# GianniLunardi/VBOC

Hardware: AMD Instinct MI355X
Metric: VBOC boundary OCP solves/sec, triple pendulum, 1/2/4/8 MI355X (higher is better)
Workload: dtype f64

## Files before the change

vboc_amd/csrc/coop.h:

```cpp
#pragma once

#ifndef VBOC_NSF
#define VBOC_NSF 4
#endif
#ifndef VBOC_DF
#define VBOC_DF 2
#endif
#ifndef VBOC_NSV
#define VBOC_NSV 8
#endif
#ifndef VBOC_DV
#define VBOC_DV 6
#endif

namespace vboc {

typedef double dbl2 __attribute__((ext_vector_type(2)));
typedef double dbl4 __attribute__((ext_vector_type(4)));
typedef __attribute__((address_space(1))) dbl2 gdbl2;
typedef __attribute__((address_space(1))) void gvoid;
typedef __attribute__((address_space(3))) void lvoid;

__host__ __device__ constexpr int even_up(int v) { return (v + 1) & ~1; }
#ifndef VBOC_REC_ALIGN
// ... 172 lines not shown
#else
#define CPROF_DECL
#define CPROF(i)
#define CPROF_FLUSH(sq, ip)
#endif
#if defined(VBOC_COOP_PROF) && defined(VBOC_PROF_SPLIT)
#define SPROF_DECL(P) unsigned long long sp0 = 0, sp1 = 0, sp2 = 0, sp3 = 0, sp4 = 0, sp_t = 0; \
  constexpr bool sp_on = (VBOC_PROF_SPLIT == (P)); if (sp_on) sp_t = __builtin_amdgcn_s_memtime();
#define SPROF(i) if (sp_on) { const unsigned long long n_ = __builtin_amdgcn_s_memtime(); sp##i += n_ - sp_t; sp_t = n_; }
#define SPROF_FLUSH if (sp_on && t == 0) { atomicAdd(&g_wave_prof[11], sp0); atomicAdd(&g_wave_prof[12], sp1); \
  atomicAdd(&g_wave_prof[13], sp2); atomicAdd(&g_wave_prof[14], sp3); atomicAdd(&g_wave_prof[15], sp4); }
#else
#define SPROF_DECL(P)
#define SPROF(i)
#define SPROF_FLUSH
#endif
#ifndef VBOC_REPEAT
#define VBOC_REPEAT 0
#endif

#define VREP(id, stmt) do { stmt; if constexpr (VBOC_REPEAT == (id)) { stmt; } } while (0)

#ifndef VBOC_FUSE
#define VBOC_FUSE 31
#endif

template <int NQ, bool FM = false, bool HC = false>
struct Coop {
  using L = WaveLayout<NQ>;
  using HL = Lane<NQ>;
  static_assert(!HC || (!FM && NQ >= 2 && NQ <= 3), "path constraint: pendulum chains, VALU factorisation");
  using PF = Par<NQ>;
  static constexpr int NX = 2 * NQ, NU = NQ, NZ = 3 * NQ, M0 = NQ + 1, REC = L::REC;
  static constexpr bool FUSE_OK = FM && NQ <= 3 && !HC;
  static constexpr bool FAC1 = FUSE_OK && (VBOC_FUSE & 1), PFUSE = FUSE_OK && (VBOC_FUSE & 2),
                        CCORR = FUSE_OK && (VBOC_FUSE & 4), KFM = FUSE_OK && (VBOC_FUSE & 8);
  static constexpr int OA = L::OA, OB = L::OB, OZ = L::OZ, ODZ = L::ODZ, OQL = L::OQL, OQU = L::OQU,
                       OE = L::OE, OK = L::OK, OKF = L::OKF, OLR = L::OLR, OM = L::OM, OY = L::OY,
                       OPE = L::OPE, OD = L::OD, ODA = L::ODA, OC = L::OC, OACL = L::OACL, OX = L::OX, OU = L::OU,
                       OPI = L::OPI,
                       OLL = L::OLL, OLU = L::OLU, OWPI = L::OWPI;

  double* s;
  gdouble* g;
  const Work& w;
  const Opts& o;
  int t;
  int N;
  double rs, rd0, e00, mu, nbox;

  unsigned lds0;
  gdouble* gh = nullptr;
  int pause_at = -1;

  __device__ Coop(double* s_, gdouble* g_, const Work& w_, const Opts& o_, int t_)
      : s(s_), g(g_), w(w_), o(o_), t(t_), N(0),
        lds0((unsigned)__builtin_amdgcn_readfirstlane((int)(unsigned)(size_t)(lvoid*)s_)) {}

  __device__ __forceinline__ void fresh() { asm volatile("" : "+v"(t)); }
// ... 104 lines not shown
  __device__ __forceinline__ double cgrad(int k, int i) const { return (k == 0 && i == 0) ? par(PF::CS) : 0.0; }

  template <int LO, int C>
  __device__ __forceinline__ void ldr(int k, double (&d)[2 * C]) const {
    static_assert(LO % 2 == 0, "16-byte aligned range");
    const gdbl2* src = (const gdbl2*)(g + (long long)k * REC + LO);
    UNR for (int c = 0; c < C; ++c) {
      const dbl2 v = src[c];
      d[2 * c] = v.x;
      d[2 * c + 1] = v.y;
    }
  }
  static constexpr int NIP = (4 * NZ + 1) / 2;
  struct IP { double v[2 * NIP]; };
  __device__ __forceinline__ void ld_ip(int k, IP& r) const { ldr<OZ, NIP>(k, r.v); }
  template <int LO, int CNT, bool WIDE = !L::IN_FIRST>
  struct Cov {
    static_assert(LO >= OD && LO + CNT <= OD + 2 * NZ, "a part of the D / DA slots");
    static constexpr int B = WIDE ? OD : (LO & ~1), OFF = LO - B, C = WIDE ? (2 * NZ + 1) / 2 : (OFF + CNT + 1) / 2;
    double v[2 * C];
  };
  template <int LO, int CNT>
  __device__ __forceinline__ void ldc(int k, Cov<LO, CNT>& c) const { ldr<Cov<LO, CNT>::B, Cov<LO, CNT>::C>(k, c.v); }

  struct CS { double tl, tu, itl, itu, ql, qu, dz; bool bx; };
  __device__ __forceinline__ CS comp_r(const IP& r, int k, int i) const {
    CS c;
    double lb, ub;
    c.bx = box(k, i, lb, ub);
    const double z = r.v[i];
    c.dz = r.v[NZ + i]; c.ql = r.v[2 * NZ + i]; c.qu = r.v[3 * NZ + i];
    c.tl = c.dz - (lb - z); c.tu = (ub - z) - c.dz;
    c.itl = c.bx ? 1.0 / c.tl : 0.0;
    c.itu = c.bx ? 1.0 / c.tu : 0.0;
    return c;
  }
  __device__ __forceinline__ CS comp(int k, int i) const {
    CS c;
    double lb, ub;
    c.bx = box(k, i, lb, ub);
    const double z = st(k, OZ + i);
    c.dz = st(k, ODZ + i); c.ql = st(k, OQL + i); c.qu = st(k, OQU + i);
    c.tl = c.dz - (lb - z); c.tu = (ub - z) - c.dz;
    c.itl = c.bx ? 1.0 / c.tl : 0.0;
    c.itu = c.bx ? 1.0 / c.tu : 0.0;
    return c;
// ... 421 lines not shown
    for (int k = t; k <= N; k += 64) {
      IP r;
      ld_ip(k, r);
      __builtin_amdgcn_sched_barrier(0);
      gdouble* rec = &g[(long long)k * REC];
      prep_from(r, k, rec);
      if constexpr (HC) {
        if (hc_on(k)) {
          const double htl = hcr(k, HL::HTL), htu = hcr(k, HL::HTU), hql = hcr(k, HL::HQL), hqu = hcr(k, HL::HQU);
          const double sig = hql / htl + hqu / htu;
          const double gam = hql * (rs * hcr(k, HL::HR0L)) / htl - hqu * (rs * hcr(k, HL::HR0U)) / htu;
          double hg[NQ];
          UNR for (int j = 0; j < NQ; ++j) hg[j] = hcr(k, HL::HG + j);
          UNR for (int i = 0; i < NQ; ++i) {
            UNR for (int j = 0; j < NQ; ++j)
              rec[OK + i * NQ + j] = (i == j ? (double)rec[OD + i] : 0.0) + sig * hg[i] * hg[j];
            rec[ODA + i] += hg[i] * gam;
          }
        }
      }
    }
    __syncthreads();
  }
  __device__ __forceinline__ void prep_corr(double smu) {
    fresh();
    for (int k = t; k <= N; k += 64) {
      IP r;
      Cov<ODA, NZ> da;
      ld_ip(k, r);
      ldc(k, da);
      __builtin_amdgcn_sched_barrier(0);
      gdouble* rec = &g[(long long)k * REC];
      double gv[NZ];
      UNR for (int i = 0; i < NZ; ++i) {
        const CS c = comp_r(r, k, i);
        double gg = o.lm * c.dz + cgrad(k, i);
        if (c.bx) {
          double rl, ru;
          corr_rhs(c, da.v[da.OFF + i], smu, rl, ru);
          gg += -c.ql - rl * c.itl + c.qu + ru * c.itu;
        }
        rec[OD + i] = gg;
        gv[i] = gg;
      }
      if constexpr (CCORR) {
        if (k >= 1 && k < N) vec_const(k, gv);
      }
      if constexpr (HC) {
// ... 578 lines not shown
        double x = st(0, OG + a);
        UNR for (int i = 0; i < NX; ++i) x += s[L::F0 + i * M0 + a] * v[i];
        w0[a] = x;
      }
      UNR for (int e = 0; e < M0 * M0; ++e) Lm[e] = s[L::LR0 + e];
      chol_solve<M0>(Lm, w0);
      UNR for (int a = 0; a < M0; ++a) w0[a] = -w0[a];
      UNR for (int j = 0; j < NQ; ++j)
        UNR for (int a = 0; a < M0; ++a) lin[j] += s[L::Y0 + a * NQ + j] * w0[a];
    }
    double Sl[NQ * NQ];
    UNR for (int e = 0; e < NQ * NQ; ++e) Sl[e] = s[L::SC + e];
    const bool ok = chol<NQ>(Sl);
    UNR for (int j = 0; j < NQ; ++j) nun[j] = lin[j] + s[L::LINE + j] - rs * par(PF::E0N + j);
    chol_solve<NQ>(Sl, nun);
    __syncthreads();
    SPROF(3)
    SPROF_FLUSH
    return ok;
  }

  template <bool CORR>
  __device__ __forceinline__ void fwd(const double (&w0in)[M0], const double (&nun)[NQ], double smu, double& amax, double& c0,
                      double& c1, double& c2) {
    fresh();
    constexpr int OT = CORR ? OD : ODA;
#if defined(VBOC_PROF_SPLIT) && VBOC_PROF_SPLIT == 6
    constexpr int WSPL = 6;
#else
    constexpr int WSPL = 3;
#endif
#define W3(i) if constexpr (WSPL == 3) { SPROF(i) }
#define W6(i) if constexpr (WSPL == 6) { SPROF(i) }
    SPROF_DECL(WSPL)
    {
      double w0[M0];
      UNR for (int a = 0; a < M0; ++a) {
        double x = w0in[a];
        UNR for (int j = 0; j < NQ; ++j) x -= s[L::MM0 + a * NQ + j] * nun[j];
        w0[a] = x;
      }
      if (t == 0) {
        UNR for (int i = 0; i < NZ; ++i) st(0, OT + i) = i < M0 ? w0[i < M0 ? i : 0] : 0.0;

      }
      if (t < NX) {
        double x = rs * st(0, OE + t);
// ... 101 lines not shown
        const int k = 1 + j;
        wdma(j + L::DV);
        vmwait<(L::DV - 1) * PW>();
        double an[NX], cn;
        fld(vslot((j + 1) % L::NSV), an, cn);
        __builtin_amdgcn_sched_barrier(0);
        double p0 = cc, p1 = 0.0;
        UNR for (int q = 0; q < NX; q += 2) p0 += acl[q] * dx[q];
        UNR for (int q = 1; q < NX; q += 2) p1 += acl[q] * dx[q];
        const double dn = p0 + p1;
        if (t < NX) s[L::XS + (k + 1) * NX + t] = dn;
        UNR for (int q = 0; q < NX; ++q) dx[q] = rdlane(dn, q);
        UNR for (int q = 0; q < NX; ++q) acl[q] = an[q];
        cc = cn;
      }
    }
    }
    __syncthreads();
    W3(2)
    W6(4)
    typename Lane<NQ>::MinRatio mr{1.0, CORR ? o.tau : 1.0};
    double a0 = 0.0, a1 = 0.0, a2 = 0.0;
    constexpr int NKM = KFM ? (OKF + NU - OK + 1) / 2 : (OY - OK + 1) / 2;
    for (int k = t; k <= N; k += 64) {
      IP r;
      double km[2 * NKM];
      Cov<ODA, NZ> da;
      const int kk = (k > 0 && k < N) ? k : 1 < N ? 1 : 0;
      ld_ip(k, r);
      ldr<OK, NKM>(kk, km);
      if (CORR) ldc(k, da);
      __builtin_amdgcn_sched_barrier(0);
      W6(0)
      gdouble* rec = &g[(long long)k * REC];
      double d[NZ];
      if (k == 0) {
        UNR for (int i = 0; i < NZ; ++i) d[i] = rec[OT + i];
      } else {
        UNR for (int i = 0; i < NX; ++i) d[i] = s[L::XS + k * NX + i];
        UNR for (int a = 0; a < NU; ++a) {
          double x = 0.0;
          if (k < N) {
            x = km[OKF - OK + a];
            if constexpr (!KFM) {
              UNR for (int j = 0; j < NQ; ++j) x -= km[OM - OK + a * NQ + j] * nun[j];
            }
// ... 34 lines not shown
            hcr(k, HL::HATL) = dtl; hcr(k, HL::HATU) = dtu; hcr(k, HL::HAQL) = dql; hcr(k, HL::HAQU) = dqu;
            a0 += htl * hql + htu * hqu;
            a1 += htl * dql + dtl * hql + htu * dqu + dtu * hqu;
            a2 += dtl * dql + dtu * dqu;
          }
          mr.add(htl, dtl);
          mr.add(htu, dtu);
          mr.add(hql, dql);
          mr.add(hqu, dqu);
        }
      }
      W6(2)
    }
    amax = wmind(mr.value());
    c0 = wsum(a0); c1 = wsum(a1); c2 = wsum(a2);
    __syncthreads();
    W3(3)
    W6(3)
    SPROF_FLUSH
#undef W3
#undef W6
  }

  __device__ __forceinline__ void update(double alpha, double smu) {
    fresh();
    double musum = 0.0;
    for (int k = t; k <= N; k += 64) {
      IP r;
      double dd[2 * ((2 * NZ + 1) / 2)];
      ld_ip(k, r);
      ldr<OD, (2 * NZ + 1) / 2>(k, dd);
      __builtin_amdgcn_sched_barrier(0);
      gdouble* rec = &g[(long long)k * REC];
      IP rn;
      if constexpr (PFUSE) rn = r;
      UNR for (int i = 0; i < NZ; ++i) {
        const CS c = comp_r(r, k, i);
        const double d = dd[i];
        const double dzn = c.dz + alpha * d;
        rec[ODZ + i] = dzn;
        if constexpr (PFUSE) rn.v[NZ + i] = dzn;
        if (!c.bx) continue;
        double rl, ru;
        corr_rhs(c, dd[NZ + i], smu, rl, ru);
        const double dll = (rl - c.ql * d) * c.itl, dlu = (ru + c.qu * d) * c.itu;
        const double qln = c.ql + alpha * dll, qun = c.qu + alpha * dlu;
        rec[OQL + i] = qln;
// ... 233 lines not shown
      else if (rstat < o.tol_stat && req < o.tol_eq && rineq < o.tol_ineq && rcomp < o.tol_comp) status = 0;
      else if (it >= o.max_iter) status = 2;
      if (status >= 0) break;
      qp_init();
      CPROF(1)
      int qcur = 0, qst = 1;
      double w0[M0], nun[NQ];
      for (;;) {
        int q = qp_check();
        if (q == 1 && qcur >= o.qp_max_iter) q = 2;
        if (q != 1) { qst = q; break; }
        if (!PFUSE || qcur == 0) VREP(1, prep_pred());
        CPROF(2)
        bool okf;
        if constexpr (FM) VREP(2, okf = factor_mfma());
        else VREP(2, okf = factor());
        if constexpr (!ACL_FUSED) VREP(3, acl_pass());
        CPROF(3)
        bool okv;
        VREP(4, (okv = vec<ODA, true, VFUSE>(w0, nun)));
        CPROF(4)
        if (!(okf && okv)) { qst = -1; break; }
        double aa, c0, c1, c2;
        VREP(5, fwd<false>(w0, nun, 0.0, aa, c0, c1, c2));
        CPROF(5)
        const double muaff = (c0 + aa * (c1 + aa * c2)) / nbox;
        double sig = muaff / mu;
        sig = fmin(1.0, sig * sig * sig);
        const double smu = sig * mu;
        VREP(6, prep_corr(smu));
        CPROF(2)
        bool okc;
        VREP(7, (okc = vec<OD, !CCORR>(w0, nun)));
        if (!okc) { qst = -1; break; }
        CPROF(4)
        double amax;
        VREP(8, fwd<true>(w0, nun, smu, amax, c0, c1, c2));
        CPROF(5)
        const double alpha = fmin(1.0, o.tau * amax);
        update(alpha, smu);
        if (t == 0) {
          UNR for (int j = 0; j < NQ; ++j) par(PF::QNU + j) += alpha * (nun[j] - par(PF::QNU + j));
        }
        __syncthreads();
        rs *= (1.0 - alpha);
        ++qcur;
        CPROF(6)
      }
      qit += qcur;
      qtot += qcur;
      if (qst < 0 || !costate()) { status = 4; break; }
      CPROF(7)
      update_weights();
      double alpha = 1.0;
      const double phi0 = merit(0.0);
      for (;;) {
        const double pa = merit(alpha);
        if (pa < phi0) break;
        if (alpha * o.alpha_red < o.alpha_min) break;
        alpha *= o.alpha_red;
      }
      apply(alpha);
      CPROF(8)
// ... 54 lines not shown
            in.sqp_iter[pid] = 0;
            in.qp_iter[pid] = 0;
            atomicAdd(ss.done, 1u);
          }
          continue;
        }
      }
      C.from_inputs(in, pid);
    }
    const int status = C.run(it, qit);
    C.store(in, pid, status, it, qit);
    __syncthreads();
    if (t == 0) {
      if (jb.list) {
        ss(IS_PID, slot) = -1;
        ss(IS_PH, slot) = 0;
      }
      atomicAdd(ss.done, 1u);
    }
  }
  if constexpr (NQ == 3 && FM && !HC && Coop<NQ, FM, HC>::VFUSE) asm volatile(".rept 96\n\ts_nop 0\n\t.endr");
}

__global__ void k_list(SlotState ss, int* list, unsigned* cnt) {
  const unsigned slot = blockIdx.x * blockDim.x + threadIdx.x;
  if (ss(IS_PID, slot) >= 0 && ss(IS_PH, slot) == 1) list[atomicAdd(cnt, 1u)] = (int)slot;
}

}
```

vboc_amd/csrc/dg.h:

```cpp
#pragma once

namespace vboc {

struct DgJobs {
  const long long* ids;
  int count;
  int N_start, nmax;
  int fail_mod;
  int max_restarts;
  double fmt_scale;
  unsigned long long seed;
  double q_min, q_max, v_max, u_max, dt, tol, eps, g, l1, l2, m1, m2;
  double* xs;
  double* us;
  double* vr;
  double* st;
  int vr_cap, st_doubles;
  double* rows;
  long long rows_cap;
  long long* row_off;
  int* row_cnt;
  double* ic;
  int* ic_slot;
  double* stats;
// ... 899 lines not shown
    const int e = ld_flag(&J->park_q[(long long)q * J->count + h]);
    if (e > 0 && (unsigned)(e - 1) / (unsigned)J->round_n < r) return true;
  }
  return false;
}
template <int NQ>
__device__ __forceinline__ bool dg_restart_before(const DgJobs* J, unsigned r) {
  const unsigned h = __hip_atomic_load(J->spec_q_head, __ATOMIC_RELAXED, __HIP_MEMORY_SCOPE_AGENT);
  if (h >= __hip_atomic_load(J->spec_q_tail, __ATOMIC_RELAXED, __HIP_MEMORY_SCOPE_AGENT)) return false;
  const int e = ld_flag(&J->spec_q[h]);
  if (e <= 0) return false;
  after_flag();
  const int ev = (e - 1) / (DG_SPEC_JOBS + 1);
  const double job = ld_coh(J->spec + (long long)ev * J->spec_stride + Dg<NQ>::H_JOB);
  return (unsigned)job / (unsigned)J->round_n < r;
}

template <int NQ, bool FM>
__global__ __launch_bounds__(64) __attribute__((amdgpu_waves_per_eu(WavesPerEu<NQ>::v, WavesPerEu<NQ>::v)))
void k_dg(Work w, Opts o, Inputs in, const Inputs* inp, const DgJobs* J, WaveJobs jb) {
  extern __shared__ __attribute__((aligned(16))) double smem[];
  const int t = (int)threadIdx.x;
  const int wg = (int)blockIdx.x;
  Coop<NQ, FM> C(smem, gptr(jb.regions) + (long long)wg * jb.region_doubles, w, o, t);
  const int count = J->count;
  const bool spec = J->spec_events > 0;
  const bool park = J->park_res != nullptr;
  if (spec && J->spec_crit && t == 0) {
    unsigned long long z = 0;
    __hip_atomic_compare_exchange_strong(J->t_launch, &z, (unsigned long long)__builtin_amdgcn_s_memrealtime(),
                                         __ATOMIC_RELAXED, __ATOMIC_RELAXED, __HIP_MEMORY_SCOPE_AGENT);
  }
  for (;;) {
    int mode = 0, idx = 0, ev = 0, jj = 0, code = 0;
    if (spec && (J->spec_window > 0 || J->spec_crit)) {
      int got = -1;
      if (t == 0) {
        const unsigned h = __hip_atomic_load(J->spec_eq_head, __ATOMIC_RELAXED, __HIP_MEMORY_SCOPE_AGENT);
        unsigned hh = h;
        if (h < __hip_atomic_load(J->spec_eq_tail, __ATOMIC_RELAXED, __HIP_MEMORY_SCOPE_AGENT) &&
            __hip_atomic_compare_exchange_strong(J->spec_eq_head, &hh, h + 1, __ATOMIC_RELAXED, __ATOMIC_RELAXED,
                                                 __HIP_MEMORY_SCOPE_AGENT)) {
          int e;
          while ((e = ld_flag(&J->spec_eq[h])) == 0) __builtin_amdgcn_s_sleep(2);
          after_flag();
          const int ev_ = (e - 1) / (DG_SPEC_JOBS + 1), jj_ = (e - 1) % (DG_SPEC_JOBS + 1);
          if (ld_flag(&J->spec_cancel[ev_]) == 0 &&
// ... 381 lines not shown

template <int NQ>
__device__ __forceinline__ bool ts_start(const DgJobs* J, const Inputs* in, int wg, int t, int job) {
  Ts<NQ> T(*J, *in, wg, t);
  return T.start(job);
}
template <int NQ>
__device__ __forceinline__ int ts_feed(const DgJobs* J, const Inputs* in, int wg, int t, int job) {
  Ts<NQ> T(*J, *in, wg, t);
  return T.feed(job);
}
template <int NQ>
__device__ __forceinline__ void ts_finish(const DgJobs* J, const Inputs* in, int wg, int t, int job) {
  Ts<NQ> T(*J, *in, wg, t);
  T.finish(job);
}

template <int NQ, bool FM>
__global__ __launch_bounds__(64) __attribute__((amdgpu_waves_per_eu(WavesPerEu<NQ>::v, WavesPerEu<NQ>::v)))
void k_ts(Work w, Opts o, Inputs in, const Inputs* inp, const DgJobs* J, WaveJobs jb) {
  extern __shared__ __attribute__((aligned(16))) double smem[];
  const int t = (int)threadIdx.x;
  const int wg = (int)blockIdx.x;
  Coop<NQ, FM> C(smem, gptr(jb.regions) + (long long)wg * jb.region_doubles, w, o, t);
  const int count = J->count;
  for (;;) {
    int got = -1;
    if (t == 0 && __hip_atomic_load(jb.next, __ATOMIC_RELAXED, __HIP_MEMORY_SCOPE_AGENT) < (unsigned)count) {
      const unsigned i = atomicAdd(jb.next, 1u);
      if (i < (unsigned)count) got = (int)i;
    }
    got = dg_bcast(got);
    if (got < 0) break;
    int code = ts_start<NQ>(J, inp, wg, t, got) ? 1 : 0;
    while (code) {
      __syncthreads();
      int it = 0, qit = 0;
      Lane<NQ> chk(w, o, 0u);
      if (!chk.supported(in, wg)) {
        if (t == 0) {
          in.status[wg] = 5;
          in.sqp_iter[wg] = 0;
          in.qp_iter[wg] = 0;
        }
      } else {
        C.from_inputs(in, wg);
        const int status = C.run(it, qit);
// ... 228 lines not shown
```

vboc_amd/csrc/vboc_solver.hip:

```cpp
#include <hip/hip_runtime.h>

#include <chrono>
#include <cmath>
#include <cstdlib>
#include <cstdio>
#include <cstring>
#include <string>
#include <vector>

#include "../../include/vboc.h"
#include "model.h"

#define UNR _Pragma("unroll")
#ifdef VBOC_WAVES
#define VBOC_WPE __attribute__((amdgpu_waves_per_eu(VBOC_WAVES, VBOC_WAVES)))
#else
#define VBOC_WPE
#endif

namespace vboc {

struct Opts {
  double tol_stat, tol_eq, tol_ineq, tol_comp;
  double qp_tol_stat, qp_tol_eq, qp_tol_comp;
// ... 1317 lines not shown
  int nq, nmax, device;
  long long slots;
  Opts o;
  Work w;
  void* pool = nullptr;
  size_t pool_bytes = 0;
  unsigned int* head = nullptr;
  int* ist = nullptr;
  unsigned int* host_done = nullptr;
  hipEvent_t ev0 = nullptr, ev1 = nullptr;
  int launches = 0;
  bool profile = false;
  std::vector<hipEvent_t> pev;
  int npev = 0;
  double fact_ms = 0.0;
  long long fact_calls = 0;
  unsigned long long fact_stages = 0;
  void* stage = nullptr;
  size_t stage_bytes = 0;
  int* list = nullptr;
  double coop_threshold = 8192;
  bool wave_all = true;
  bool factor_mfma = true;
  double* regions = nullptr;
  long long n_regions = 0, region_doubles = 0, group_cap = 0;
  double mall_mib = 256.0;
  size_t wave_lds = 0;
  bool coop_ok = false;
  long long coop_count = 0;
  double* ft_regions = nullptr;
  size_t ft_bytes = 0;
  double* dg_scratch = nullptr;
  size_t dg_bytes = 0;
  DgJobs* dg_jobs = nullptr;
  Inputs* dg_in = nullptr;
  TtJobs* tt_jobs = nullptr;
  bool tt_attr[2] = {false, false};
  bool dg_attr[4] = {false, false, false, false};
  int dg_fail_mod = 0;
  bool dg_speculate = true;
  int dg_spec_early = 0;
  int dg_spec_pause = 300;
  int dg_spec_first = 2;
  bool dg_spec_crit = false;
  int dg_spec_window = 0;
  double* wave_hc = nullptr;
// ... 112 lines not shown
    h->ft_bytes = need;
  }
  if constexpr (NQ == 3) {
    if (mp.on) {
      hipLaunchKernelGGL((k_ft<NQ, true>), dim3((unsigned)groups), dim3(64), 0, st, h->o, in, h->ft_regions, rd, h->head,
                         mp);
      return hipGetLastError() == hipSuccess ? 0 : -2;
    }
  }
  if (mp.on) return -2;
  hipLaunchKernelGGL((k_ft<NQ, false>), dim3((unsigned)groups), dim3(64), 0, st, h->o, in, h->ft_regions, rd, h->head,
                     mp);
  return hipGetLastError() == hipSuccess ? 0 : -2;
}

static long long wave_group_budget(const vboc_solver* h, int nmax) {
  const long long hot = (long long)(h->nq == 1 ? WaveLayout<1>::OX
                                    : (h->nq == 2 ? WaveLayout<2>::OX : (h->nq == 3 ? WaveLayout<3>::OX : WaveLayout<4>::OX))) *
                        (long long)(nmax + 1) * (long long)sizeof(double);
  const long long g = (long long)(0.92 * h->mall_mib * 1024.0 * 1024.0) / (hot > 0 ? hot : 1);
  return g < 256 ? 256 : g;
}

static hipError_t launch_wave(vboc_solver* h, const WaveJobs& jb, long long jobs, hipStream_t st, const Work& w,
                              const Inputs& in, const SlotState& ss) {
  long long groups = jobs < h->n_regions ? jobs : h->n_regions;
  const long long cap = h->group_cap > 0 ? h->group_cap : (h->mall_mib > 0 ? wave_group_budget(h, in.nmax) : 0);
  if (cap > 0 && groups > cap) groups = cap;
  if (groups < 1) return hipSuccess;
  h->last_groups = groups;
  const dim3 grid((unsigned)groups), block(64);
  switch (h->nq) {
    case 1:
      if (h->factor_mfma) hipLaunchKernelGGL((k_wave<1, true>), grid, block, h->wave_lds, st, w, h->o, in, ss, jb);
      else hipLaunchKernelGGL((k_wave<1, false>), grid, block, h->wave_lds, st, w, h->o, in, ss, jb);
      break;
    case 2:
      if (h->o.hc) hipLaunchKernelGGL((k_wave<2, false, true>), grid, block, h->wave_lds, st, w, h->o, in, ss, jb);
      else if (h->factor_mfma) hipLaunchKernelGGL((k_wave<2, true>), grid, block, h->wave_lds, st, w, h->o, in, ss, jb);
      else hipLaunchKernelGGL((k_wave<2, false>), grid, block, h->wave_lds, st, w, h->o, in, ss, jb);
      break;
    case 3:
      if (h->factor_mfma) hipLaunchKernelGGL((k_wave<3, true>), grid, block, h->wave_lds, st, w, h->o, in, ss, jb);
      else hipLaunchKernelGGL((k_wave<3, false>), grid, block, h->wave_lds, st, w, h->o, in, ss, jb);
      break;
    default: hipLaunchKernelGGL((k_wave<4, false>), grid, block, h->wave_lds, st, w, h->o, in, ss, jb); break;
  }
  return hipGetLastError();
}

template <int NQ, bool FM>
static hipError_t launch_dg(vboc_solver* h, const DgJobs& J, const Inputs& in, long long groups, hipStream_t st,
                           bool testing = false) {
  const void* fn = testing ? (const void*)k_ts<NQ, FM> : (const void*)k_dg<NQ, FM>;
  bool& attr = h->dg_attr[(FM ? 1 : 0) + (testing ? 2 : 0)];
  if (!attr) {
    hipError_t e = hipFuncSetAttribute(fn, hipFuncAttributeMaxDynamicSharedMemorySize, (int)h->wave_lds);
    if (e != hipSuccess) return e;
    attr = true;
  }
  WaveJobs jb{nullptr, J.count, J.next, h->regions, h->region_doubles};
  hipError_t e = hipMemcpyAsync(h->dg_jobs, &J, sizeof(DgJobs), hipMemcpyHostToDevice, st);
  if (e == hipSuccess) e = hipMemcpyAsync(h->dg_in, &in, sizeof(Inputs), hipMemcpyHostToDevice, st);
  if (e == hipSuccess) e = hipStreamSynchronize(st);
  if (e != hipSuccess) return e;
  if (testing)
// ... 157 lines not shown
  if (!h || !f) return fail(VBOC_ERR_ARG, "vboc_set_option: NULL argument");
  Opts& o = h->o;
  const std::string s(f);
  if (s == "nlp_solver_tol_stat") o.tol_stat = v;
  else if (s == "nlp_solver_tol_eq") o.tol_eq = v;
  else if (s == "nlp_solver_tol_ineq") o.tol_ineq = v;
  else if (s == "nlp_solver_tol_comp") o.tol_comp = v;
  else if (s == "nlp_solver_max_iter") o.max_iter = (int)v;
  else if (s == "qp_solver_iter_max") o.qp_max_iter = (int)v;
  else if (s == "qp_solver_tol_stat") o.qp_tol_stat = v;
  else if (s == "qp_solver_tol_eq") o.qp_tol_eq = v;
  else if (s == "qp_solver_tol_comp") o.qp_tol_comp = v;
  else if (s == "levenberg_marquardt") o.lm = v;
  else if (s == "alpha_min") o.alpha_min = v;
  else if (s == "alpha_reduction") o.alpha_red = v;
  else if (s == "ipm_mu0") o.mu0 = v;
  else if (s == "ipm_push") o.push = v;
  else if (s == "ipm_tau") o.tau = v;
  else if (s == "coop_threshold") h->coop_threshold = v;
  else if (s == "wave_all") {
    h->wave_all = v != 0.0;
  }
  else if (s == "factor_mfma") h->factor_mfma = v != 0.0 && h->nq <= 3;
  else if (s == "wave_groups") h->group_cap = (long long)v;
  else if (s == "mall_mib") h->mall_mib = v;
  else if (s == "dg_fail_mod") h->dg_fail_mod = (int)v;
  else if (s == "dg_speculate") h->dg_speculate = v != 0.0;
  else if (s == "dg_spec_early") h->dg_spec_early = v > 0.0 ? (int)v : 0;
  else if (s == "dg_spec_pause") h->dg_spec_pause = v > 0.0 ? (int)v : 0;
  else if (s == "dg_spec_first") h->dg_spec_first = v >= 2.0 ? 2 : (v != 0.0 ? 1 : 0);
  else if (s == "dg_spec_crit") h->dg_spec_crit = v != 0.0;
  else if (s == "dg_spec_window") h->dg_spec_window = v > 0.0 ? (v < 9.0 ? (int)v : 9) : 0;
  else if (s == "dg_park") h->dg_park = v != 0.0;
  else if (s == "dg_park_window") h->dg_park_window = v > 0.0 ? (int)v : 0;
  else if (s == "dg_park_hi") h->dg_park_hi = v > 0.0 ? (int)v : 0;
  else if (s == "dg_round") h->dg_round = v > 0.0 ? (int)v : 0;
  else if (s == "hc_wave") h->hc_wave = v != 0.0;
  else if (s == "profile_kernels") {
    h->profile = v != 0.0;
    if (h->profile && h->pev.empty()) {
      h->pev.resize(2 * 4096);
      for (auto& ev : h->pev)
        if (hipEventCreate(&ev) != hipSuccess) return fail(VBOC_ERR_HIP, "vboc_set_option: hipEventCreate");
    }
  } else return fail(VBOC_ERR_ARG, "vboc_set_option: unknown field '" + s + "'");
  return VBOC_OK;
// ... 13 lines not shown
  else if (s == "qp_solver_tol_eq") *v = o.qp_tol_eq;
  else if (s == "qp_solver_tol_comp") *v = o.qp_tol_comp;
  else if (s == "levenberg_marquardt") *v = o.lm;
  else if (s == "alpha_min") *v = o.alpha_min;
  else if (s == "alpha_reduction") *v = o.alpha_red;
  else if (s == "ipm_mu0") *v = o.mu0;
  else if (s == "ipm_push") *v = o.push;
  else if (s == "ipm_tau") *v = o.tau;
  else if (s == "coop_threshold") *v = h->coop_threshold;
  else if (s == "coop_available") *v = h->coop_ok ? 1.0 : 0.0;
  else if (s == "wave_all") *v = h->wave_all ? 1.0 : 0.0;
  else if (s == "dg_speculate") *v = h->dg_speculate ? 1.0 : 0.0;
  else if (s == "dg_spec_early") *v = (double)h->dg_spec_early;
  else if (s == "dg_spec_pause") *v = (double)h->dg_spec_pause;
  else if (s == "dg_spec_first") *v = (double)h->dg_spec_first;
  else if (s == "dg_spec_crit") *v = h->dg_spec_crit ? 1.0 : 0.0;
  else if (s == "dg_spec_window") *v = (double)h->dg_spec_window;
  else if (s == "dg_park") *v = h->dg_park ? 1.0 : 0.0;
  else if (s == "dg_park_window") *v = (double)h->dg_park_window;
  else if (s == "dg_park_hi") *v = (double)h->dg_park_hi;
  else if (s == "dg_round") *v = (double)h->dg_round;
  else if (s == "hc_wave") *v = h->hc_wave ? 1.0 : 0.0;
  else if (s == "factor_mfma") *v = h->factor_mfma ? 1.0 : 0.0;
  else if (s == "wave_groups") *v = (double)h->n_regions;
  else if (s == "last_groups") *v = (double)h->last_groups;
  else if (s == "dg_busy") *v = h->dg_busy ? 1.0 : 0.0;
  else if (s == "mall_mib") *v = h->mall_mib;
  else if (s == "coop_problems") *v = (double)h->coop_count;
  else if (s == "slots") *v = (double)h->slots;
  else if (s == "workspace_bytes") *v = (double)h->pool_bytes;
  else return fail(VBOC_ERR_ARG, "vboc_get_option: unknown field '" + s + "'");
  return VBOC_OK;
}

int vboc_set_path_constraint(vboc_handle h, int kind, double x_c, double y_c, double lh, double uh) {
  if (busy(h, "vboc_set_path_constraint")) return VBOC_ERR_ARG;
  if (!h) return fail(VBOC_ERR_ARG, "vboc_set_path_constraint: NULL handle");
  if (kind == 0) { h->o.hc = 0; return VBOC_OK; }
  if (kind != 1) return fail(VBOC_ERR_ARG, "vboc_set_path_constraint: unknown kind");
  if (h->nq != 2 && h->nq != 3)
    return fail(VBOC_ERR_UNSUPPORTED, "vboc_set_path_constraint: the keep-out circle needs a pendulum chain (nq 2 or 3)");
  if (!(lh <= uh)) return fail(VBOC_ERR_ARG, "vboc_set_path_constraint: lh > uh");
  if (!h->w.HC) {
    const size_t f = h->nq == 2 ? (size_t)Lane<2>::FHC : (size_t)Lane<3>::FHC;
    HIPCHK(hipSetDevice(h->device));
    const hipError_t e = hipMalloc((void**)&h->w.HC, sizeof(double) * ev(f) * (size_t)(h->nmax + 1) * (size_t)h->slots);
// ... 680 lines not shown
  HIPCHK(hipStreamSynchronize(st));
  const unsigned* c = h->host_done;
  if (c[3]) return fail(VBOC_ERR_ARG, "vboc_testing_test: a horizon passed the handle's nmax");
  if (c[1] != (unsigned)b->B) return fail(VBOC_ERR_HIP, "vboc_testing_test: not every problem finished");
  return VBOC_OK;
}

static int dg_wait(vboc_handle h, vboc_dg_batch_t* b, hipStream_t st) {
  hipError_t e = hipSetDevice(h->device);
  if (e == hipSuccess) e = hipMemcpyAsync(h->host_done, h->head, 14 * sizeof(unsigned), hipMemcpyDeviceToHost, st);
  if (e == hipSuccess) e = hipStreamSynchronize(st);
  h->dg_busy = false;
  if (e != hipSuccess) return fail(VBOC_ERR_HIP, std::string("vboc_data_generation: waiting for the launch: ") + hipGetErrorString(e));
  const unsigned* c = h->host_done;
  b->rows_used = (long long)(((unsigned long long)c[5] << 32) | c[4]);
  b->spec_solves = (long long)(((unsigned long long)c[11] << 32) | c[10]);
  b->spec_used = (long long)(((unsigned long long)c[13] << 32) | c[12]);
  if (c[2]) return fail(VBOC_ERR_NOMEM, "vboc_data_generation: the row pool (rows_cap) overflowed");
  if (c[3]) return fail(VBOC_ERR_HIP, "vboc_data_generation: a horizon exceeded nmax (internal error)");
  if (c[1] != (unsigned)b->B) return fail(VBOC_ERR_HIP, "vboc_data_generation: not every problem finished");
  return VBOC_OK;
}

int vboc_hjr_solve_batch(vboc_handle h, const vboc_hjr_batch_t* b, void* stream) {
  if (busy(h, "vboc_hjr_solve_batch")) return VBOC_ERR_ARG;
  if (!h || !b) return fail(VBOC_ERR_ARG, "vboc_hjr_solve_batch: NULL argument");
  if (h->nq > 3) return fail(VBOC_ERR_UNSUPPORTED, "vboc_hjr_solve_batch: defined for the pendulum chains (nq 1-3)");
  if (b->B < 0) return fail(VBOC_ERR_ARG, "vboc_hjr_solve_batch: B < 0");
  if (b->B == 0) return VBOC_OK;
  if (b->hidden != 100)
    return fail(VBOC_ERR_UNSUPPORTED, "vboc_hjr_solve_batch: NeuralNetCLS hidden size 100 (the reference's) only");
  if (!b->x0 || !b->W0 || !b->b0 || !b->W1 || !b->b1 || !b->W2 || !b->b2 || !b->status || !b->cost || !b->u ||
      !b->x1 || !b->sqp_iter || !b->qp_iter)
    return fail(VBOC_ERR_ARG, "vboc_hjr_solve_batch: NULL array");
  if (!(b->std > 0.0) || !(b->u_max > 0.0)) return fail(VBOC_ERR_ARG, "vboc_hjr_solve_batch: std and u_max must be > 0");
  HIPCHK(hipSetDevice(h->device));
  hipStream_t st = (hipStream_t)stream;
  Opts o;
  default_opts(o);
  o.tol_stat = 1e-6;
  o.qp_tol_stat = 1e-8;
  o.lm = h->nq == 1 ? 1e-2 : 1e-5;
  HjrNet net{b->W0, b->b0, b->W1, b->b1, b->W2, b->b2, b->mean, b->std};
  HjrJobs J{b->B, b->x0, b->u_max, b->status, b->cost, b->u, b->x1, b->sqp_iter, b->qp_iter};
  const dim3 grid((unsigned)((b->B + 63) / 64)), block(64);
  HIPCHK(hipEventRecord(h->ev0, st));
// ... 78 lines not shown
```

Before: 20330.

## Carry last-trip stage registers across forward/correction/update passes in wave solver

Adds an interior-point carry path in the cooperative wave solver for the triple pendulum. The last trip of the forward sweep keeps its loaded record, direction and covariance slots in registers and hands them to prep_corr and update, which process that trip first without reloading it from global memory. The correction forward pass runs its trips in reverse order so the carried trip lines up with update's first trip. A new k_wave_ic kernel and a wave_carry option, on by default, route nq=3 MFMA solves through this path. The cost is higher register pressure from the carried state, which may lower occupancy.

```diff
diff --git a/vboc_amd/csrc/coop.h b/vboc_amd/csrc/coop.h
--- a/vboc_amd/csrc/coop.h
+++ b/vboc_amd/csrc/coop.h
@@ -218,10 +218,16 @@
 #define VREP(id, stmt) do { stmt; if constexpr (VBOC_REPEAT == (id)) { stmt; } } while (0)
 
 #ifndef VBOC_FUSE
-#define VBOC_FUSE 31
+#define VBOC_FUSE 63
 #endif
-
-template <int NQ, bool FM = false, bool HC = false>
+#ifndef VBOC_ICARRY_NQ
+#define VBOC_ICARRY_NQ (1 << 3)
+#endif
+#ifndef VBOC_ICARRY_PAIRS
+#define VBOC_ICARRY_PAIRS 2
+#endif
+
+template <int NQ, bool FM = false, bool HC = false, bool IC = false>
 struct Coop {
   using L = WaveLayout<NQ>;
   using HL = Lane<NQ>;
@@ -230,7 +236,9 @@
   static constexpr int NX = 2 * NQ, NU = NQ, NZ = 3 * NQ, M0 = NQ + 1, REC = L::REC;
   static constexpr bool FUSE_OK = FM && NQ <= 3 && !HC;
   static constexpr bool FAC1 = FUSE_OK && (VBOC_FUSE & 1), PFUSE = FUSE_OK && (VBOC_FUSE & 2),
-                        CCORR = FUSE_OK && (VBOC_FUSE & 4), KFM = FUSE_OK && (VBOC_FUSE & 8);
+                        CCORR = FUSE_OK && (VBOC_FUSE & 4), KFM = FUSE_OK && (VBOC_FUSE & 8),
+                        ICARRY = IC && FUSE_OK && (VBOC_FUSE & 32) && ((VBOC_ICARRY_NQ >> NQ) & 1),
+                        ICA = ICARRY && (VBOC_ICARRY_PAIRS & 1), ICB = ICARRY && (VBOC_ICARRY_PAIRS & 2);
   static constexpr int OA = L::OA, OB = L::OB, OZ = L::OZ, ODZ = L::ODZ, OQL = L::OQL, OQU = L::OQU,
                        OE = L::OE, OK = L::OK, OKF = L::OKF, OLR = L::OLR, OM = L::OM, OY = L::OY,
                        OPE = L::OPE, OD = L::OD, ODA = L::ODA, OC = L::OC, OACL = L::OACL, OX = L::OX, OU = L::OU,
@@ -381,6 +389,16 @@
   };
   template <int LO, int CNT>
   __device__ __forceinline__ void ldc(int k, Cov<LO, CNT>& c) const { ldr<Cov<LO, CNT>::B, Cov<LO, CNT>::C>(k, c.v); }
+  struct Carry { IP r; double d[NZ]; Cov<ODA, NZ> da; };
+  template <bool DA>
+  __device__ __forceinline__ static void taken(Carry& c) {
+    UNR for (int i = 0; i < 2 * NIP; ++i) asm volatile("" : "+v"(c.r.v[i]));
+    UNR for (int i = 0; i < NZ; ++i) asm volatile("" : "+v"(c.d[i]));
+    if constexpr (DA) {
+      UNR for (int i = 0; i < (int)(sizeof(c.da.v) / sizeof(double)); ++i) asm volatile("" : "+v"(c.da.v[i]));
+    }
+  }
+  __device__ __forceinline__ int trips() const { return (N + 64) >> 6; }
 
   struct CS { double tl, tu, itl, itu, ql, qu, dz; bool bx; };
   __device__ __forceinline__ CS comp_r(const IP& r, int k, int i) const {
@@ -848,8 +866,42 @@
     }
     __syncthreads();
   }
-  __device__ __forceinline__ void prep_corr(double smu) {
+  __device__ __forceinline__ void prep_corr(double smu, const Carry& cyin) {
     fresh();
+    if constexpr (ICA) {
+      Carry cy = cyin;
+      taken<false>(cy);
+      auto stage = [&](int k, const IP& r, const double* da) __attribute__((always_inline)) {
+        gdouble* rec = &g[(long long)k * REC];
+        double gv[NZ];
+        UNR for (int i = 0; i < NZ; ++i) {
+          const CS c = comp_r(r, k, i);
+          double gg = o.lm * c.dz + cgrad(k, i);
+          if (c.bx) {
+            double rl, ru;
+            corr_rhs(c, da[i], smu, rl, ru);
+            gg += -c.ql - rl * c.itl + c.qu + ru * c.itu;
+          }
+          rec[OD + i] = gg;
+          gv[i] = gg;
+        }
+        if constexpr (CCORR) {
+          if (k >= 1 && k < N) vec_const(k, gv);
+        }
+      };
+      const int kl = t + 64 * (trips() - 1);
+      if (kl <= N) stage(kl, cy.r, cy.d);
+      for (int k = t; k < kl; k += 64) {
+        IP r;
+        Cov<ODA, NZ> da;
+        ld_ip(k, r);
+        ldc(k, da);
+        __builtin_amdgcn_sched_barrier(0);
+        stage(k, r, da.v + da.OFF);
+      }
+      __syncthreads();
+      return;
+    }
     for (int k = t; k <= N; k += 64) {
       IP r;
       Cov<ODA, NZ> da;
@@ -1474,7 +1526,7 @@
 
   template <bool CORR>
   __device__ __forceinline__ void fwd(const double (&w0in)[M0], const double (&nun)[NQ], double smu, double& amax, double& c0,
-                      double& c1, double& c2) {
+                      double& c1, double& c2, Carry& cy) {
     fresh();
     constexpr int OT = CORR ? OD : ODA;
 #if defined(VBOC_PROF_SPLIT) && VBOC_PROF_SPLIT == 6
@@ -1622,6 +1674,72 @@
     typename Lane<NQ>::MinRatio mr{1.0, CORR ? o.tau : 1.0};
     double a0 = 0.0, a1 = 0.0, a2 = 0.0;
     constexpr int NKM = KFM ? (OKF + NU - OK + 1) / 2 : (OY - OK + 1) / 2;
+    if constexpr (CORR ? ICB : ICA) {
+      const int nt = trips();
+      auto trip = [&](int j, Carry& cc) __attribute__((always_inline)) {
+        const int kq = t + 64 * (CORR ? nt - 1 - j : j);
+        const bool own = kq <= N;
+        const int k = own ? kq : N;
+        IP& r = cc.r;
+        double (&d)[NZ] = cc.d;
+        Cov<ODA, NZ>& da = cc.da;
+        double km[2 * NKM];
+        const int kk = (k > 0 && k < N) ? k : 1 < N ? 1 : 0;
+        ld_ip(k, r);
+        ldr<OK, NKM>(kk, km);
+        if (CORR) ldc(k, da);
+        __builtin_amdgcn_sched_barrier(0);
+        W6(0)
+        gdouble* rec = &g[(long long)k * REC];
+        if (k == 0) {
+          UNR for (int i = 0; i < NZ; ++i) d[i] = rec[OT + i];
+        } else {
+          UNR for (int i = 0; i < NX; ++i) d[i] = s[L::XS + k * NX + i];
+          UNR for (int a = 0; a < NU; ++a) {
+            double x = 0.0;
+            if (k < N) {
+              x = km[OKF - OK + a];
+              if constexpr (!KFM) {
+                UNR for (int j2 = 0; j2 < NQ; ++j2) x -= km[OM - OK + a * NQ + j2] * nun[j2];
+              }
+              UNR for (int i = 0; i < NX; ++i) x += km[a * NX + i] * d[i];
+            }
+            d[NX + a] = x;
+          }
+          if (own) {
+            UNR for (int i = 0; i < NZ; ++i) rec[OT + i] = d[i];
+          }
+        }
+        W6(1)
+        UNR for (int i = 0; i < NZ; ++i) {
+          const CS c = comp_r(r, k, i);
+          if (!c.bx || !own) continue;
+          double dll, dlu;
+          if (!CORR) {
+            dll = -c.ql - c.ql * d[i] * c.itl;
+            dlu = -c.qu + c.qu * d[i] * c.itu;
+            a0 += c.tl * c.ql + c.tu * c.qu;
+            a1 += c.tl * dll + d[i] * c.ql + c.tu * dlu - d[i] * c.qu;
+            a2 += d[i] * dll - d[i] * dlu;
+          } else {
+            double rl, ru;
+            corr_rhs(c, da.v[da.OFF + i], smu, rl, ru);
+            dll = (rl - c.ql * d[i]) * c.itl;
+            dlu = (ru + c.qu * d[i]) * c.itu;
+          }
+          mr.add(c.tl, d[i]);
+          mr.add(c.tu, -d[i]);
+          mr.add(c.ql, dll);
+          mr.add(c.qu, dlu);
+        }
+        W6(2)
+      };
+      for (int j = 0; j < nt - 1; ++j) {
+        Carry loc;
+        trip(j, loc);
+      }
+      trip(nt - 1, cy);
+    } else
     for (int k = t; k <= N; k += 64) {
       IP r;
       double km[2 * NKM];
@@ -1702,7 +1820,47 @@
 #undef W6
   }
 
-  __device__ __forceinline__ void update(double alpha, double smu) {
+  __device__ __forceinline__ void update(double alpha, double smu, const Carry& cyin) {
+    if constexpr (ICB) {
+      fresh();
+      Carry cy = cyin;
+      taken<true>(cy);
+      double musum = 0.0;
+      auto stage = [&](int k, const IP& r, const double* dv, const double* da) __attribute__((always_inline)) {
+        gdouble* rec = &g[(long long)k * REC];
+        IP rn;
+        if constexpr (PFUSE) rn = r;
+        UNR for (int i = 0; i < NZ; ++i) {
+          const CS c = comp_r(r, k, i);
+          const double d = dv[i];
+          const double dzn = c.dz + alpha * d;
+          rec[ODZ + i] = dzn;
+          if constexpr (PFUSE) rn.v[NZ + i] = dzn;
+          if (!c.bx) continue;
+          double rl, ru;
+          corr_rhs(c, da[i], smu, rl, ru);
+          const double dll = (rl - c.ql * d) * c.itl, dlu = (ru + c.qu * d) * c.itu;
+          const double qln = c.ql + alpha * dll, qun = c.qu + alpha * dlu;
+          rec[OQL + i] = qln;
+          rec[OQU + i] = qun;
+          if constexpr (PFUSE) { rn.v[2 * NZ + i] = qln; rn.v[3 * NZ + i] = qun; }
+          musum += (c.tl + alpha * d) * qln + (c.tu - alpha * d) * qun;
+        }
+        if constexpr (PFUSE) prep_from(rn, k, rec);
+      };
+      if (t <= N) stage(t, cy.r, cy.d, cy.da.v + cy.da.OFF);
+      for (int k = t + 64; k <= N; k += 64) {
+        IP r;
+        double dd[2 * ((2 * NZ + 1) / 2)];
+        ld_ip(k, r);
+        ldr<OD, (2 * NZ + 1) / 2>(k, dd);
+        __builtin_amdgcn_sched_barrier(0);
+        stage(k, r, dd, dd + NZ);
+      }
+      mu = wsum(musum) / nbox;
+      __syncthreads();
+      return;
+    }
     fresh();
     double musum = 0.0;
     for (int k = t; k <= N; k += 64) {
@@ -1982,23 +2140,24 @@
         CPROF(4)
         if (!(okf && okv)) { qst = -1; break; }
         double aa, c0, c1, c2;
-        VREP(5, fwd<false>(w0, nun, 0.0, aa, c0, c1, c2));
+        Carry cy;
+        VREP(5, fwd<false>(w0, nun, 0.0, aa, c0, c1, c2, cy));
         CPROF(5)
         const double muaff = (c0 + aa * (c1 + aa * c2)) / nbox;
         double sig = muaff / mu;
         sig = fmin(1.0, sig * sig * sig);
         const double smu = sig * mu;
-        VREP(6, prep_corr(smu));
+        VREP(6, prep_corr(smu, cy));
         CPROF(2)
         bool okc;
         VREP(7, (okc = vec<OD, !CCORR>(w0, nun)));
         if (!okc) { qst = -1; break; }
         CPROF(4)
         double amax;
-        VREP(8, fwd<true>(w0, nun, smu, amax, c0, c1, c2));
+        VREP(8, fwd<true>(w0, nun, smu, amax, c0, c1, c2, cy));
         CPROF(5)
         const double alpha = fmin(1.0, o.tau * amax);
-        update(alpha, smu);
+        update(alpha, smu, cy);
         if (t == 0) {
           UNR for (int j = 0; j < NQ; ++j) par(PF::QNU + j) += alpha * (nun[j] - par(PF::QNU + j));
         }
@@ -2099,6 +2258,53 @@
   if constexpr (NQ == 3 && FM && !HC && Coop<NQ, FM, HC>::VFUSE) asm volatile(".rept 96\n\ts_nop 0\n\t.endr");
 }
 
+template <int NQ, bool FM>
+__global__ __launch_bounds__(64) __attribute__((amdgpu_waves_per_eu(WavesPerEu<NQ>::v, WavesPerEu<NQ>::v)))
+void k_wave_ic(Work w, Opts o, Inputs in, SlotState ss, WaveJobs jb) {
+  extern __shared__ __attribute__((aligned(16))) double smem[];
+  const int t = (int)threadIdx.x;
+  Coop<NQ, FM, false, true> C(smem, gptr(jb.regions) + (long long)blockIdx.x * jb.region_doubles, w, o, t);
+  for (;;) {
+    unsigned idx = 0;
+    if (t == 0) idx = atomicAdd(jb.next, 1u);
+    idx = (unsigned)__builtin_amdgcn_readfirstlane((int)__shfl((int)idx, 0));
+    if (idx >= (unsigned)jb.count) break;
+    int pid, it = 0, qit = 0;
+    unsigned slot = 0;
+    if (jb.list) {
+      slot = (unsigned)__builtin_amdgcn_readfirstlane(jb.list[idx]);
+      pid = ss(IS_PID, slot);
+      it = ss(IS_IT, slot);
+      qit = ss(IS_QIT, slot);
+      C.from_slot(ss, slot);
+    } else {
+      pid = (int)idx;
+      Lane<NQ> chk(w, o, 0u);
+      if (!chk.supported(in, pid)) {
+        if (t == 0) {
+          in.status[pid] = 5;
+          in.cost[pid] = NAN;
+          in.sqp_iter[pid] = 0;
+          in.qp_iter[pid] = 0;
+          atomicAdd(ss.done, 1u);
+        }
+        continue;
+      }
+      C.from_inputs(in, pid);
+    }
+    const int status = C.run(it, qit);
+    C.store(in, pid, status, it, qit);
+    __syncthreads();
+    if (t == 0) {
+      if (jb.list) {
+        ss(IS_PID, slot) = -1;
+        ss(IS_PH, slot) = 0;
+      }
+      atomicAdd(ss.done, 1u);
+    }
+  }
+}
+
 __global__ void k_list(SlotState ss, int* list, unsigned* cnt) {
   const unsigned slot = blockIdx.x * blockDim.x + threadIdx.x;
   if (ss(IS_PID, slot) >= 0 && ss(IS_PH, slot) == 1) list[atomicAdd(cnt, 1u)] = (int)slot;
diff --git a/vboc_amd/csrc/dg.h b/vboc_amd/csrc/dg.h
--- a/vboc_amd/csrc/dg.h
+++ b/vboc_amd/csrc/dg.h
@@ -945,7 +945,7 @@
   extern __shared__ __attribute__((aligned(16))) double smem[];
   const int t = (int)threadIdx.x;
   const int wg = (int)blockIdx.x;
-  Coop<NQ, FM> C(smem, gptr(jb.regions) + (long long)wg * jb.region_doubles, w, o, t);
+  Coop<NQ, FM, false, true> C(smem, gptr(jb.regions) + (long long)wg * jb.region_doubles, w, o, t);
   const int count = J->count;
   const bool spec = J->spec_events > 0;
   const bool park = J->park_res != nullptr;
@@ -1373,7 +1373,7 @@
   extern __shared__ __attribute__((aligned(16))) double smem[];
   const int t = (int)threadIdx.x;
   const int wg = (int)blockIdx.x;
-  Coop<NQ, FM> C(smem, gptr(jb.regions) + (long long)wg * jb.region_doubles, w, o, t);
+  Coop<NQ, FM, false, true> C(smem, gptr(jb.regions) + (long long)wg * jb.region_doubles, w, o, t);
   const int count = J->count;
   for (;;) {
     int got = -1;
diff --git a/vboc_amd/csrc/vboc_solver.hip b/vboc_amd/csrc/vboc_solver.hip
--- a/vboc_amd/csrc/vboc_solver.hip
+++ b/vboc_amd/csrc/vboc_solver.hip
@@ -1363,6 +1363,7 @@
   double coop_threshold = 8192;
   bool wave_all = true;
   bool factor_mfma = true;
+  bool wave_carry = true;
   double* regions = nullptr;
   long long n_regions = 0, region_doubles = 0, group_cap = 0;
   double mall_mib = 256.0;
@@ -1521,6 +1522,9 @@
   return g < 256 ? 256 : g;
 }
 
+static void launch_wave_ic(const dim3& grid, const dim3& block, size_t lds, hipStream_t st, const Work& w, const Opts& o,
+                           const Inputs& in, const SlotState& ss, const WaveJobs& jb);
+
 static hipError_t launch_wave(vboc_solver* h, const WaveJobs& jb, long long jobs, hipStream_t st, const Work& w,
                               const Inputs& in, const SlotState& ss) {
   long long groups = jobs < h->n_regions ? jobs : h->n_regions;
@@ -1540,7 +1544,8 @@
       else hipLaunchKernelGGL((k_wave<2, false>), grid, block, h->wave_lds, st, w, h->o, in, ss, jb);
       break;
     case 3:
-      if (h->factor_mfma) hipLaunchKernelGGL((k_wave<3, true>), grid, block, h->wave_lds, st, w, h->o, in, ss, jb);
+      if (h->factor_mfma && h->wave_carry) launch_wave_ic(grid, block, h->wave_lds, st, w, h->o, in, ss, jb);
+      else if (h->factor_mfma) hipLaunchKernelGGL((k_wave<3, true>), grid, block, h->wave_lds, st, w, h->o, in, ss, jb);
       else hipLaunchKernelGGL((k_wave<3, false>), grid, block, h->wave_lds, st, w, h->o, in, ss, jb);
       break;
     default: hipLaunchKernelGGL((k_wave<4, false>), grid, block, h->wave_lds, st, w, h->o, in, ss, jb); break;
@@ -1744,6 +1749,7 @@
     h->wave_all = v != 0.0;
   }
   else if (s == "factor_mfma") h->factor_mfma = v != 0.0 && h->nq <= 3;
+  else if (s == "wave_carry") h->wave_carry = v != 0.0;
   else if (s == "wave_groups") h->group_cap = (long long)v;
   else if (s == "mall_mib") h->mall_mib = v;
   else if (s == "dg_fail_mod") h->dg_fail_mod = (int)v;
@@ -1803,6 +1809,7 @@
   else if (s == "dg_round") *v = (double)h->dg_round;
   else if (s == "hc_wave") *v = h->hc_wave ? 1.0 : 0.0;
   else if (s == "factor_mfma") *v = h->factor_mfma ? 1.0 : 0.0;
+  else if (s == "wave_carry") *v = h->wave_carry ? 1.0 : 0.0;
   else if (s == "wave_groups") *v = (double)h->n_regions;
   else if (s == "last_groups") *v = (double)h->last_groups;
   else if (s == "dg_busy") *v = h->dg_busy ? 1.0 : 0.0;
@@ -2529,6 +2536,15 @@
   return VBOC_OK;
 }
 
+}
+
+static void launch_wave_ic(const dim3& grid, const dim3& block, size_t lds, hipStream_t st, const Work& w, const Opts& o,
+                           const Inputs& in, const SlotState& ss, const WaveJobs& jb) {
+  hipLaunchKernelGGL((k_wave_ic<3, true>), grid, block, lds, st, w, o, in, ss, jb);
+}
+
+extern "C" {
+
 int vboc_hjr_solve_batch(vboc_handle h, const vboc_hjr_batch_t* b, void* stream) {
   if (busy(h, "vboc_hjr_solve_batch")) return VBOC_ERR_ARG;
   if (!h || !b) return fail(VBOC_ERR_ARG, "vboc_hjr_solve_batch: NULL argument");
```

Result: no change. 20420, median of 3 (+0.5%).
